# HanielUlises/GCN-GrabCut

Measured on AMD Instinct MI355X. Metric: images/sec end-to-end mask (DUTS-shape batch), higher is better.
Workload: dtype f32

## Files before the change

### gcn-grabcut_amd/csrc/ggc_internal.h

```cpp
#pragma once
#include <hip/hip_runtime.h>
#include <cstdint>
#include <cstdio>
#include <atomic>
#include <cstring>
#include <map>
#include <string>
#include <vector>
#include "../../include/ggc.h"
#include "../../include/ggc_fmath.h"

namespace ggc {

constexpr int WAVE = 64;

enum Slot : int {
    S_CSR_ROWPTR = 0, S_CSR_COL, S_CSR_EID, S_CSR_CURSOR, S_CSR_SCAN, S_DIS, S_BATCH, S_AGG_PACK,
    S_STATES, S_GATE, S_XW, S_AGG, S_SCORE, S_GVEC, S_HJK,
    S_PRE_A, S_PRE_B, S_PRE_C, S_PRE_D,
    S_SLIC_IMG, S_SLIC_TMP, S_SLIC_CENTERS, S_SLIC_DIST, S_SLIC_LABELS, S_SLIC_AUX,
    S_SLIC_AUX2, S_SLIC_AUX3, S_SLIC_AUX4, S_SLIC_MINMAX,
    S_G_STATS, S_G_FEAT, S_G_PAIRS, S_G_PAIRCNT, S_G_NL, S_G_EDGE_SRC, S_G_EDGE_DST,
    S_G_EDGE_ATTR, S_G_PTR, S_G_PRIOR, S_G_AUX, S_G_AUX2, S_G_AUX3, S_G_X,
    S_T_A, S_T_B, S_T_C,
    S_GC_A, S_GC_B, S_GC_C, S_GC_D, S_GC_E, S_GC_F, S_GC_G, S_GC_H, S_GC_I, S_GC_J,
    S_GC_K, S_GC_L, S_GC_M,
    S_CC_A, S_CC_B, S_CC_C,
    S_MISC_A, S_MISC_B,
    S_CLICK,
    S_MATTE, S_MATTE_MEAN, S_CFMATTE,
    S_FOREGROUND, S_FOREGROUND_VEC,
    S_MATTE_EVAL,
    S_FULLCUT,
    S_GEODESIC,
    S_STROKES,
    S_COUNT
};

struct Buf {
    void*  p = nullptr;
    size_t bytes = 0;
};

struct WeightSet {
    int D = 0;
    int Dt = 0;
    int n_layers = 0;
    int Q = 0, C = 0;
    int heads = 0;
    std::map<std::string, std::vector<float>> host;
    std::map<std::string, Buf> dev;
    bool dev_ok = false;
};

struct GraphState {
    int B = 0, H = 0, W = 0;
    int64_t n_total = 0, e_total = 0;
    std::vector<int64_t> node_ptr, edge_ptr;
    int64_t max_pairs = 0;
    int n_max = 0;
    const int32_t* n_nodes_dev = nullptr;
    bool valid = false;
};

}

namespace ggc {
struct ProfRec { const char* name; hipEvent_t a, b; };
}

struct ggc_ctx {
    int device = 0;
    std::string err;
    int prof_on = 0;
    double prof_overhead_ms = 0.0;
    std::vector<ggc::ProfRec> prof;
    std::vector<hipEvent_t> prof_pool;
    ggc::Buf slots[ggc::S_COUNT];
    ggc::WeightSet resgcn, gcnnet, gat;
    ggc::GraphState graph;
    int n_cu = 256;
    float prior_two_ce2 = (float)(2 * 0.45 * 0.45), prior_two_cs2 = (float)(2 * 0.40 * 0.40);
    int32_t* h_pinned = nullptr;
    static constexpr int H_PINNED_INTS = 4096;
};

namespace ggc {

struct Knobs {
    int mf_trace;
    int mf_warm;
    int mf_async_push_active;
    int mf_async_tile;
    int mf_async_hops;
    int mf_async_sweeps;
    int mf_dense_launches0, mf_dense_launches;
    int mf_dense_sweeps;
    int mf_relax_dense;
    int mf_partial_rounds;
    int agg_direct;
    int slic_seq_connectivity;
    int matte_eval_levels;
};
const Knobs& knobs();

int set_err(ggc_ctx* ctx, int code, const char* fmt, ...);
int read_i32(ggc_ctx* ctx, hipStream_t st, const int32_t* dev, int n, std::vector<int32_t>& host);
void* scratch(ggc_ctx* ctx, int slot, size_t bytes);
int build_csr(ggc_ctx* ctx, hipStream_t st, int N, int E, const int32_t* src, const int32_t* dst,
              int32_t* row_ptr, int32_t* col, int32_t* eid, int32_t* cursor, float* dis);

#define GGC_HIP(ctx, expr)                                                          \
    do {                                                                            \
        hipError_t _e = (expr);                                                     \
        if (_e != hipSuccess)                                                       \
            return ggc::set_err((ctx), GGC_E_DEVICE, "%s failed: %s (%s:%d)", #expr, \
                                hipGetErrorString(_e), __FILE__, __LINE__);          \
    } while (0)

#define GGC_LAUNCH_CHECK(ctx)                                                        \
    do {                                                                            \
        hipError_t _e = hipGetLastError();                                          \
        if (_e != hipSuccess)                                                       \
            return ggc::set_err((ctx), GGC_E_DEVICE, "kernel launch failed: %s (%s:%d)", \
                                hipGetErrorString(_e), __FILE__, __LINE__);          \
    } while (0)

#define GGC_REQUIRE(ctx, cond, code, ...)                      \
    do {                                                       \
        if (!(cond)) return ggc::set_err((ctx), (code), __VA_ARGS__); \
    } while (0)

template <typename T>
inline T* scratch_t(ggc_ctx* ctx, int slot, size_t count) {
    return reinterpret_cast<T*>(scratch(ctx, slot, count * sizeof(T)));
}

struct Carve {
    char* base = nullptr;
    size_t bytes = 0;
    template <typename T> T* take(size_t count) {
        T* p = base ? reinterpret_cast<T*>(base + bytes) : nullptr;
        bytes += (count * sizeof(T) + 255) & ~size_t(255);
        return p;
    }
};
template <typename Layout>
inline size_t carve_scratch(ggc_ctx* ctx, int slot, Layout&& layout) {
    Carve c;
    layout(c);
    c.base = static_cast<char*>(scratch(ctx, slot, c.bytes));
    if (!c.base) return 0;
    c.bytes = 0;
    layout(c);
    return c.bytes;
}

inline int cdiv(int64_t a, int64_t b) { return (int)((a + b - 1) / b); }

struct DeviceOnce {
    std::atomic<unsigned long long> mask{0};
    bool need(int dev) const { return dev < 0 || dev >= 64 || !((mask.load(std::memory_order_acquire) >> dev) & 1ull); }
    void done(int dev) { if (dev >= 0 && dev < 64) mask.fetch_or(1ull << dev, std::memory_order_release); }
};

struct ProfScope {
    ggc_ctx* ctx; hipStream_t st; hipEvent_t b = nullptr;
// ... 73 lines not shown
```

### gcn-grabcut_amd/csrc/ggc_math.h

```cpp
#pragma once
#include <hip/hip_runtime.h>
#include <cstdint>
#include <cstring>

namespace ggc {

__host__ __device__ inline double bits_to_double(uint64_t u) {
#if defined(__HIP_DEVICE_COMPILE__)
    return __longlong_as_double((long long)u);
#else
    double d; std::memcpy(&d, &u, 8); return d;
#endif
}
__host__ __device__ inline uint64_t double_to_bits(double d) {
#if defined(__HIP_DEVICE_COMPILE__)
    return (uint64_t)__double_as_longlong(d);
#else
    uint64_t u; std::memcpy(&u, &d, 8); return u;
#endif
}

__host__ __device__ inline double det_cbrt(double a) {
    double y = bits_to_double(double_to_bits(a) / 3 + 0x2A9F7893782DA1CEULL);
#pragma unroll
    for (int i = 0; i < 6; ++i) {
        const double y2 = y * y;
        y = y - (y2 * y - a) / (3.0 * y2);
    }
    return y;
}

__host__ __device__ inline double det_pow24(double a) {
    const double q = a * a;
    double y = bits_to_double(double_to_bits(q) / 5 + 0x3325FFFFFFFFFFFFULL);
#pragma unroll
    for (int i = 0; i < 7; ++i) {
        const double y2 = y * y;
        const double y4 = y2 * y2;
        y = y - (y4 * y - q) / (5.0 * y4);
    }
    return q * y;
}

__host__ __device__ inline double det_exp(double x) {
    const double LN2_HI = 6.93147180369123816490e-01, LN2_LO = 1.90821492927058770002e-10;
    const double INV_LN2 = 1.44269504088896338700e+00;
    if (x != x) return x;
    if (x < -745.2) return 0.0;
    if (x > 709.782712893384) return bits_to_double(0x7FF0000000000000ULL);
    const double k = rint(x * INV_LN2);
    const double r = (x - k * LN2_HI) - k * LN2_LO;
    double p = 1.0 / 6227020800.0;
    p = p * r + 1.0 / 479001600.0;
    p = p * r + 1.0 / 39916800.0;
    p = p * r + 1.0 / 3628800.0;
    p = p * r + 1.0 / 362880.0;
    p = p * r + 1.0 / 40320.0;
    p = p * r + 1.0 / 5040.0;
    p = p * r + 1.0 / 720.0;
    p = p * r + 1.0 / 120.0;
    p = p * r + 1.0 / 24.0;
    p = p * r + 1.0 / 6.0;
    p = p * r + 0.5;
    p = p * r + 1.0;
    p = p * r + 1.0;
    const long long ki = (long long)k;
    const long long k1 = ki / 2, k2 = ki - k1;
    return p * bits_to_double((uint64_t)(k1 + 1023) << 52) * bits_to_double((uint64_t)(k2 + 1023) << 52);
}

__host__ __device__ inline double det_log(double x) {
    const double LN2_HI = 6.93147180369123816490e-01, LN2_LO = 1.90821492927058770002e-10;
    if (x != x || x < 0.0) return bits_to_double(0x7FF8000000000000ULL);
    if (x == 0.0) return bits_to_double(0xFFF0000000000000ULL);
    if (x > 1.7976931348623157e308) return x;
    long long e = -1023;
    if (x < 2.2250738585072014e-308) { x = x * 18014398509481984.0; e -= 54; }
    const uint64_t u = double_to_bits(x);
    e += (long long)((u >> 52) & 0x7FF);
    double m = bits_to_double((u & 0x000FFFFFFFFFFFFFULL) | 0x3FF0000000000000ULL);
    if (m > 1.4142135623730951) { m = m * 0.5; e += 1; }
    const double f = m - 1.0;
    const double s = f / (2.0 + f);
    const double z = s * s;
    double q = 1.0 / 23.0;
    q = q * z + 1.0 / 21.0;
    q = q * z + 1.0 / 19.0;
    q = q * z + 1.0 / 17.0;
    q = q * z + 1.0 / 15.0;
    q = q * z + 1.0 / 13.0;
    q = q * z + 1.0 / 11.0;
    q = q * z + 1.0 / 9.0;
    q = q * z + 1.0 / 7.0;
    q = q * z + 1.0 / 5.0;
    q = q * z + 1.0 / 3.0;
    q = q * z + 1.0;
    const double de = (double)e;
    return de * LN2_HI + (de * LN2_LO + 2.0 * s * q);
}

}
```

### gcn-grabcut_amd/csrc/ggc_preprocess.hip

```cpp
#include "ggc_internal.h"
#include "ggc_math.h"

namespace ggc {

__device__ __forceinline__ double lab_f(double t) {
    return t > 0.008856 ? det_cbrt(t) : 7.787 * t + 16.0 / 116.0;
}

__device__ __forceinline__ int reflect101(int i, int n) {
    if (n == 1) return 0;
    if (i < 0) i = -i;
    if (i >= n) i = 2 * n - 2 - i;
    return i;
}

__device__ __forceinline__ float gray_at(const uint8_t* __restrict__ img, int W, int y, int x) {
    const uint8_t* p = img + ((size_t)y * W + x) * 3;
    return (float)((p[0] * 3735 + p[1] * 19235 + p[2] * 9798 + (1 << 14)) >> 15);
}

__global__ void __launch_bounds__(256) k_preprocess(int H, int W, const uint8_t* __restrict__ bgr,
                                                    const double* __restrict__ lut,
                                                    float* __restrict__ lab, float* __restrict__ hsv,
                                                    float* __restrict__ gray, float* __restrict__ grad) {
// ... 23 lines not shown
        double s = 0.0, h = 0.0;
        if (delta != 0.0) {
            s = delta / v;
            if (r == v) h = (g - b) / delta;
            if (g == v) h = 2.0 + (b - r) / delta;
            if (b == v) h = 4.0 + (r - g) / delta;
            h = h / 6.0;
            if (h < 0.0) h = h + 1.0;
        }
        hsv[3 * p + 0] = (float)h;
        hsv[3 * p + 1] = (float)s;
        hsv[3 * p + 2] = (float)v;
    }
    if (gray) gray[p] = (float)((b8 * 3735 + g8 * 19235 + r8 * 9798 + (1 << 14)) >> 15);
    if (grad) {
        const int ym = reflect101(y - 1, H), yp = reflect101(y + 1, H);
        const int xm = reflect101(x - 1, W), xp = reflect101(x + 1, W);
        const float a = gray_at(img, W, ym, xm), b = gray_at(img, W, ym, x), c = gray_at(img, W, ym, xp);
        const float d = gray_at(img, W, y, xm), f = gray_at(img, W, y, xp);
        const float g = gray_at(img, W, yp, xm), h = gray_at(img, W, yp, x), i = gray_at(img, W, yp, xp);
        const float gx = (c + 2.0f * f + i) - (a + 2.0f * d + g);
        const float gy = (g + 2.0f * h + i) - (a + 2.0f * b + c);
        grad[p] = sqrtf(gx * gx + gy * gy);
    }
}

}

namespace ggc {
__global__ void __launch_bounds__(256) k_convert_color8(size_t n, const uint8_t* __restrict__ bgr, int mode,
                                                        const double* __restrict__ lut, const int32_t* __restrict__ sdiv,
                                                        const int32_t* __restrict__ hdiv, uint8_t* __restrict__ out) {
    const size_t p = (size_t)blockIdx.x * blockDim.x + threadIdx.x;
    if (p >= n) return;
    const int b = bgr[3 * p + 0], g = bgr[3 * p + 1], r = bgr[3 * p + 2];
    if (mode == 0) {
        const int v = max(max(b, g), r), vmin = min(min(b, g), r), diff = v - vmin;
        const int s = (diff * sdiv[v] + (1 << 11)) >> 12;
        int h = (v == r) ? (g - b) : (v == g) ? (b - r + 2 * diff) : (r - g + 4 * diff);
        h = (h * hdiv[diff] + (1 << 11)) >> 12;
        if (h < 0) h += 180;
        out[3 * p + 0] = (uint8_t)h; out[3 * p + 1] = (uint8_t)s; out[3 * p + 2] = (uint8_t)v;
        return;
    }
    const double R = lut[r], G = lut[g], B = lut[b];
    const double X = R * 0.412453 + G * 0.357580 + B * 0.180423;
    const double Y = R * 0.212671 + G * 0.715160 + B * 0.072169;
    const double Z = R * 0.019334 + G * 0.119193 + B * 0.950227;
    const double tx = X / 0.95047, ty = Y / 1.0, tz = Z / 1.08883;
    const double fx = tx > 0.008856 ? det_cbrt(tx) : 7.787 * tx + 16.0 / 116.0;
    const double fy = ty > 0.008856 ? det_cbrt(ty) : 7.787 * ty + 16.0 / 116.0;
    const double fz = tz > 0.008856 ? det_cbrt(tz) : 7.787 * tz + 16.0 / 116.0;
    const double v[3] = {(116.0 * fy - 16.0) * 255.0 / 100.0, 500.0 * (fx - fy) + 128.0, 200.0 * (fy - fz) + 128.0};
#pragma unroll
    for (int c = 0; c < 3; ++c) {
        double q = floor(v[c] + 0.5);
        q = q < 0.0 ? 0.0 : (q > 255.0 ? 255.0 : q);
        out[3 * p + c] = (uint8_t)q;
    }
}
}

using namespace ggc;

extern "C" int ggc_preprocess(ggc_ctx* ctx, ggc_stream stream, int B, int H, int W, const uint8_t* bgr,
                              float* lab, float* hsv, float* gray, float* grad) {
    if (!ctx) return GGC_E_INVALID_ARG;
    GGC_REQUIRE(ctx, B >= 1 && H >= 1 && W >= 1, GGC_E_SHAPE, "bad shape B=%d H=%d W=%d", B, H, W);
    GGC_REQUIRE(ctx, bgr != nullptr, GGC_E_INVALID_ARG, "bgr is NULL");
    GGC_REQUIRE(ctx, B <= 65535, GGC_E_SHAPE, "batch %d exceeds the grid z limit", B);
    GGC_HIP(ctx, hipSetDevice(ctx->device));
    hipStream_t st = reinterpret_cast<hipStream_t>(stream);
    double* lut = scratch_t<double>(ctx, S_PRE_A, 256);
    if (!lut) return GGC_E_OOM;
    static thread_local double host_lut[256];
    static thread_local bool lut_ready = false;
    if (!lut_ready) {
        for (int u = 0; u < 256; ++u) {
            const double v = (double)u * (1.0 / 255.0);
            host_lut[u] = v > 0.04045 ? det_pow24((v + 0.055) / 1.055) : v / 12.92;
        }
        lut_ready = true;
    }
    GGC_HIP(ctx, hipMemcpyAsync(lut, host_lut, sizeof(host_lut), hipMemcpyHostToDevice, st));
    hipLaunchKernelGGL(k_preprocess, dim3(cdiv(W, 64), cdiv(H, 4), B), dim3(256), 0, st, H, W, bgr, lut, lab, hsv,
                       gray, grad);
    GGC_LAUNCH_CHECK(ctx);
    return GGC_OK;
}

extern "C" int ggc_convert_color8(ggc_ctx* ctx, ggc_stream stream, int64_t n_pixels, const uint8_t* bgr, int mode, uint8_t* out) {
    if (!ctx) return GGC_E_INVALID_ARG;
    GGC_REQUIRE(ctx, n_pixels >= 1 && bgr && out, GGC_E_INVALID_ARG, "bad arguments");
    GGC_REQUIRE(ctx, mode == 0 || mode == 1, GGC_E_INVALID_ARG, "mode %d: 0 = HSV, 1 = Lab", mode);
    GGC_HIP(ctx, hipSetDevice(ctx->device));
    hipStream_t st = reinterpret_cast<hipStream_t>(stream);
    double* lut = scratch_t<double>(ctx, S_PRE_A, 256);
    int32_t* tabs = scratch_t<int32_t>(ctx, S_PRE_B, 512);
    if (!lut || !tabs) return GGC_E_OOM;
    double host_lut[256];
    int32_t host_tabs[512];
    for (int u = 0; u < 256; ++u) {
        const double v = (double)u * (1.0 / 255.0);
        host_lut[u] = v > 0.04045 ? det_pow24((v + 0.055) / 1.055) : v / 12.92;
        host_tabs[u] = u ? (int32_t)rint((double)(255 << 12) / (double)u) : 0;
        host_tabs[256 + u] = u ? (int32_t)rint((double)(180 << 12) / (6.0 * (double)u)) : 0;
    }
    GGC_HIP(ctx, hipMemcpyAsync(lut, host_lut, sizeof(host_lut), hipMemcpyHostToDevice, st));
    GGC_HIP(ctx, hipMemcpyAsync(tabs, host_tabs, sizeof(host_tabs), hipMemcpyHostToDevice, st));
    GGC_HIP(ctx, hipStreamSynchronize(st));
    hipLaunchKernelGGL(k_convert_color8, dim3(cdiv((size_t)n_pixels, 256)), dim3(256), 0, st, (size_t)n_pixels, bgr, mode, lut, tabs,
                       tabs + 256, out);
    GGC_LAUNCH_CHECK(ctx);
    return GGC_OK;
}
```

### gcn-grabcut_amd/csrc/ggc_slic.hip

```cpp
#include "ggc_internal.h"
#include "ggc_math.h"
#include <cmath>
#include <vector>

namespace ggc {

__device__ __forceinline__ uint32_t f2ord(float f) {
    const uint32_t u = __float_as_uint(f);
    return (u & 0x80000000u) ? ~u : (u | 0x80000000u);
}
__device__ __forceinline__ float ord2f(uint32_t o) {
    return __uint_as_float((o & 0x80000000u) ? (o & 0x7FFFFFFFu) : ~o);
}

__global__ void k_minmax_init(int B, uint32_t* mm) {
    const int i = blockIdx.x * blockDim.x + threadIdx.x;
    if (i < B) { mm[2 * i] = 0xFFFFFFFFu; mm[2 * i + 1] = 0u; }
}

__global__ void __launch_bounds__(256) k_minmax(size_t n, const float* __restrict__ img, uint32_t* mm) {
    const float* im = img + (size_t)blockIdx.y * n;
    float lo = INFINITY, hi = -INFINITY;
    for (size_t i = (size_t)blockIdx.x * blockDim.x + threadIdx.x; i < n; i += (size_t)gridDim.x * blockDim.x) {
        const float v = im[i];
        lo = fminf(lo, v); hi = fmaxf(hi, v);
    }
    for (int o = 32; o > 0; o >>= 1) { lo = fminf(lo, __shfl_xor(lo, o, 64)); hi = fmaxf(hi, __shfl_xor(hi, o, 64)); }
    __shared__ float s_lo[4], s_hi[4];
    if ((threadIdx.x & 63) == 0) { s_lo[threadIdx.x >> 6] = lo; s_hi[threadIdx.x >> 6] = hi; }
    __syncthreads();
    if (threadIdx.x == 0) {
        lo = fminf(fminf(s_lo[0], s_lo[1]), fminf(s_lo[2], s_lo[3]));
        hi = fmaxf(fmaxf(s_hi[0], s_hi[1]), fmaxf(s_hi[2], s_hi[3]));
        atomicMin(&mm[2 * blockIdx.y], f2ord(lo));
        atomicMax(&mm[2 * blockIdx.y + 1], f2ord(hi));
    }
}

__global__ void __launch_bounds__(256) k_lab2(size_t P, const float* __restrict__ img,
                                              const uint32_t* __restrict__ mm, int rescale,
                                              float* __restrict__ out) {
    const size_t p = (size_t)blockIdx.x * blockDim.x + threadIdx.x;
    if (p >= P) return;
    const size_t base = ((size_t)blockIdx.y * P + p) * 3;
    const float mn = ord2f(mm[2 * blockIdx.y]), mx = ord2f(mm[2 * blockIdx.y + 1]);
    const float range = mx - mn;
    float lin[3];
#pragma unroll
    for (int c = 0; c < 3; ++c) {
        float v = img[base + c];
        if (rescale) { v = v - mn; if (mx != mn) v = v / range; }
        lin[c] = v > (float)0.04045 ? (float)det_pow24((double)((v + (float)0.055) / (float)1.055))
                                    : v / (float)12.92;
    }
    const float X = (lin[0] * (float)0.412453 + lin[1] * (float)0.357580) + lin[2] * (float)0.180423;
    const float Y = (lin[0] * (float)0.212671 + lin[1] * (float)0.715160) + lin[2] * (float)0.072169;
    const float Z = (lin[0] * (float)0.019334 + lin[1] * (float)0.119193) + lin[2] * (float)0.950227;
    const float t[3] = {X / (float)0.95047, Y / 1.0f, Z / (float)1.08883};
    float f[3];
#pragma unroll
    for (int c = 0; c < 3; ++c)
        f[c] = t[c] > (float)0.008856 ? (float)det_cbrt((double)t[c]) : (float)7.787 * t[c] + (float)(16.0 / 116.0);
    out[base + 0] = 116.0f * f[1] - 16.0f;
    out[base + 1] = 500.0f * (f[0] - f[1]);
    out[base + 2] = 200.0f * (f[1] - f[2]);
}

constexpr int MAX_RADIUS = 16;
struct GaussW { double w[2 * MAX_RADIUS + 1]; int r; };

__device__ __forceinline__ int reflect_sym(int i, int n) {
    if ((unsigned)i < (unsigned)n) return i;
    if (n == 1) return 0;
    const int period = 2 * n;
    i %= period; if (i < 0) i += period;
    return i < n ? i : period - 1 - i;
}

template <int AXIS, int R>
__global__ void __launch_bounds__(256) k_gauss(int H, int W, const float* __restrict__ in, GaussW g,
                                               float scale, int apply_scale, float* __restrict__ out) {
    const int col = blockIdx.x * 256 + threadIdx.x;
    if (col >= 3 * W) return;
    const int y = blockIdx.y;
    const size_t n = (size_t)H * W * 3;
    const float* im = in + (size_t)blockIdx.z * n;
    const int x = col / 3, c = col - 3 * x;
    const int l = AXIS == 0 ? y : x;
    const int len = AXIS == 0 ? H : W;
    auto at = [&](int idx) -> double {
        const int j = reflect_sym(idx, len);
        return (double)(AXIS == 0 ? im[((size_t)j * W + x) * 3 + c] : im[((size_t)y * W + j) * 3 + c]);
    };
    double tmp;
    if (R > 0) {
        constexpr int RR = R > 0 ? R : 1;
        double lo[RR], hi[RR];
        const double mid = at(l);
#pragma unroll
        for (int k = 0; k < R; ++k) { lo[k] = at(l - R + k); hi[k] = at(l + R - k); }
        tmp = mid * g.w[R];
#pragma unroll
        for (int k = 0; k < R; ++k) tmp += (lo[k] + hi[k]) * g.w[k];
    } else {
        tmp = at(l) * g.w[g.r];
        for (int jj = -g.r; jj < 0; ++jj) tmp += (at(l + jj) + at(l - jj)) * g.w[jj + g.r];
    }
    float v = (float)tmp;
    if (apply_scale) v = v * scale;
    out[(size_t)blockIdx.z * n + (size_t)y * W * 3 + col] = v;
}

constexpr int GV_ROWS = 20;
template <int R>
__global__ void __launch_bounds__(256) k_gauss_v(int H, int W, const float* __restrict__ in, GaussW g, float* __restrict__ out) {
    const int col = blockIdx.x * 256 + threadIdx.x;
    if (col >= 3 * W) return;
    const size_t n = (size_t)H * W * 3;
    const float* im = in + (size_t)blockIdx.z * n + col;
    float* o = out + (size_t)blockIdx.z * n + col;
    const int y0 = blockIdx.y * GV_ROWS;
    double v[2 * R + 1];
#pragma unroll
    for (int j = 0; j < 2 * R; ++j) v[j + 1] = (double)im[(size_t)reflect_sym(y0 - R + j, H) * W * 3];
#pragma unroll 4
    for (int y = y0; y < min(y0 + GV_ROWS, H); ++y) {
#pragma unroll
        for (int j = 0; j < 2 * R; ++j) v[j] = v[j + 1];
        v[2 * R] = (double)im[(size_t)reflect_sym(y + R, H) * W * 3];
        double tmp = v[R] * g.w[R];
#pragma unroll
        for (int k = 0; k < R; ++k) tmp += (v[k] + v[2 * R - k]) * g.w[k];
        o[(size_t)y * W * 3] = (float)tmp;
    }
}

__global__ void __launch_bounds__(256) k_scale(size_t n, const float* __restrict__ in, float scale,
                                               float* __restrict__ out) {
    const size_t i = (size_t)blockIdx.x * blockDim.x + threadIdx.x;
    if (i < n) out[i] = in[i] * scale;
}

struct SlicGeom {
    int H, W, K;
    int ny, nx, start_y, start_x, step_y, step_x;
    int win_y, win_x;
    float sw;
};

__device__ __forceinline__ int4 slic_window(float cy, float cx, const SlicGeom& g) {
    if (cy != cy || cx != cx) return make_int4(0, 0, 0, 0);
    float fy0 = cy - (float)(2 * g.win_y); if (!(fy0 > 0.0f)) fy0 = 0.0f;
    float fy1 = cy + (float)(2 * g.win_y) + 1.0f; if (!(fy1 < (float)g.H)) fy1 = (float)g.H;
    float fx0 = cx - (float)(2 * g.win_x); if (!(fx0 > 0.0f)) fx0 = 0.0f;
    float fx1 = cx + (float)(2 * g.win_x) + 1.0f; if (!(fx1 < (float)g.W)) fx1 = (float)g.W;
    return make_int4((int)fy0, (int)fy1, (int)fx0, (int)fx1);
}

__global__ void k_init_centers(SlicGeom g, float* __restrict__ centers, int4* __restrict__ bounds) {
    const int k = blockIdx.x * blockDim.x + threadIdx.x;
    if (k >= g.K) return;
    const size_t o = (size_t)blockIdx.y * g.K + k;
    const float cy = (float)(g.start_y + (k / g.nx) * g.step_y);
    const float cx = (float)(g.start_x + (k % g.nx) * g.step_x);
    centers[o * 5 + 0] = cy; centers[o * 5 + 1] = cx;
    centers[o * 5 + 2] = 0.0f; centers[o * 5 + 3] = 0.0f; centers[o * 5 + 4] = 0.0f;
    bounds[o] = slic_window(cy, cx, g);
}

struct Cand { int k, y0, y1, x0, x1; float cy, cx, c0, c1, c2; };

constexpr int TILE_W = 32, TILE_H = 16;

typedef float v2f __attribute__((ext_vector_type(2)));

__global__ void __launch_bounds__(256) k_slic_assign(SlicGeom g, const float* __restrict__ image,
                                                     const float* __restrict__ centers,
                                                     const int4* __restrict__ bounds,
                                                     int32_t* __restrict__ labels, int32_t* __restrict__ stale) {
    __shared__ Cand cand[256];
    __shared__ int wcount[4];
    const int tid = threadIdx.x, lane = tid & 63, wave = tid >> 6;
    const int b = blockIdx.z;
    const int tx0 = blockIdx.x * TILE_W, ty0 = blockIdx.y * TILE_H;
    const int px = tx0 + (wave & 1) * 16 + (lane & 15), pya = ty0 + (wave >> 1) * 8 + (lane >> 4), pyb = pya + 4;
    const bool ina = px < g.W && pya < g.H, inb = px < g.W && pyb < g.H;
    const size_t P = (size_t)g.H * g.W;
    const size_t pa = (size_t)b * P + (size_t)pya * g.W + px, pb = pa + (size_t)4 * g.W;
    v2f i0 = 0.f, i1 = 0.f, i2 = 0.f;
    if (ina) { i0.x = image[3 * pa]; i1.x = image[3 * pa + 1]; i2.x = image[3 * pa + 2]; }
    if (inb) { i0.y = image[3 * pb]; i1.y = image[3 * pb + 1]; i2.y = image[3 * pb + 2]; }
    const v2f fy = {(float)pya, (float)pyb};
    const float fx = (float)px;
    float best_a = INFINITY, best_b = INFINITY;
    int lab_a = -1, lab_b = -1;
    const float* cen = centers + (size_t)b * g.K * 5;
    const int4* bnd = bounds + (size_t)b * g.K;
    for (int base = 0; base < g.K; base += 256) {
        const int k = base + tid;
        bool hit = false;
        int4 bd = make_int4(0, 0, 0, 0);
        if (k < g.K) {
            bd = bnd[k];
            hit = bd.x < ty0 + TILE_H && bd.y > ty0 && bd.z < tx0 + TILE_W && bd.w > tx0 && bd.y > bd.x && bd.w > bd.z;
        }
        const unsigned long long bal = __ballot(hit);
        const int pre = __popcll(bal & ((1ull << lane) - 1ull));
        if (lane == 0) wcount[wave] = __popcll(bal);
        __syncthreads();
        int off = 0, total = 0;
#pragma unroll
        for (int w = 0; w < 4; ++w) { if (w < wave) off += wcount[w]; total += wcount[w]; }
        if (hit) {
            Cand c;
            c.k = k; c.y0 = bd.x; c.y1 = bd.y; c.x0 = bd.z; c.x1 = bd.w;
            c.cy = cen[k * 5 + 0]; c.cx = cen[k * 5 + 1];
// ... 399 lines not shown
    return g;
}

}

using namespace ggc;

static int enforce_connectivity(ggc_ctx* ctx, hipStream_t st, int B, int H, int W, const int32_t* raw, int min_size,
                                int max_size, int32_t* segments, int32_t* n_nodes) {
    const size_t P = (size_t)H * W;
    if (knobs().slic_seq_connectivity) {
        int32_t* queue = scratch_t<int32_t>(ctx, S_SLIC_AUX3, (size_t)B * (size_t)std::max(max_size, 1));
        if (!queue) return GGC_E_OOM;
        GGC_HIP(ctx, hipMemsetAsync(segments, 0xFF, sizeof(int32_t) * (size_t)B * P, st));
        ProfScope prof(ctx, st, "slic_connectivity");
        hipLaunchKernelGGL(k_connectivity_seq, dim3(B), dim3(64), 0, st, H, W, raw, min_size, max_size, queue, segments,
                           n_nodes);
        GGC_LAUNCH_CHECK(ctx);
        return GGC_OK;
    }
    {
        ProfScope prof(ctx, st, "slic_connectivity");
        const size_t BP = (size_t)B * P;
        const CnDims cd{B, H, W, (int)P, min_size, std::max(max_size, 1)};
        int32_t* work = scratch_t<int32_t>(ctx, S_SLIC_AUX3, BP * 6 + (size_t)B * (size_t)cd.max_size + 2 * (size_t)B + 16);
        uint8_t* pending = scratch_t<uint8_t>(ctx, S_SLIC_AUX4, BP);
        if (!work || !pending) return GGC_E_OOM;
        int32_t *parent = work, *csize = work + BP, *rank = work + 2 * BP, *tgt = work + 3 * BP, *mark = work + 4 * BP;
        int32_t* queue = work + 5 * BP;
        int32_t* qtop = work + 6 * BP + (size_t)B * cd.max_size;
        int32_t* n_big = qtop + B;
        GGC_HIP(ctx, hipMemsetAsync(pending, 1, BP, st));
        GGC_HIP(ctx, hipMemsetAsync(mark, 0, sizeof(int32_t) * BP, st));
        const dim3 g1(cdiv(BP, 256)), g2(cdiv(W, 64), cdiv(H, 4), B), g64(cdiv(BP, 64));
        for (int round = 0; round < 4096; ++round) {
            GGC_HIP(ctx, hipMemsetAsync(qtop, 0, sizeof(int32_t) * (B + 1), st));
            hipLaunchKernelGGL(k_cn_reset, g1, dim3(256), 0, st, cd, raw, pending, parent, csize);
            hipLaunchKernelGGL(k_cn_merge, g2, dim3(256), 0, st, cd, raw, pending, parent);
            hipLaunchKernelGGL(k_cn_size, g1, dim3(256), 0, st, cd, raw, pending, parent, csize);
            hipLaunchKernelGGL(k_cn_settle, g1, dim3(256), 0, st, cd, pending, parent, csize, n_big);
            GGC_LAUNCH_CHECK(ctx);
            int32_t h_big = 0;
            GGC_HIP(ctx, hipMemcpyAsync(&h_big, n_big, sizeof(int32_t), hipMemcpyDeviceToHost, st));
            GGC_HIP(ctx, hipStreamSynchronize(st));
            if (h_big == 0) break;
            hipLaunchKernelGGL(k_cn_carve, g64, dim3(64), 0, st, cd, round + 1, pending, parent, csize, mark, queue, qtop);
            GGC_LAUNCH_CHECK(ctx);
        }
        hipLaunchKernelGGL(k_cn_kept, g1, dim3(256), 0, st, cd, parent, csize, rank);
        hipLaunchKernelGGL(k_cn_scan, dim3(B), dim3(1024), 0, st, cd, rank, n_nodes);
        GGC_HIP(ctx, hipMemsetAsync(qtop, 0, sizeof(int32_t) * (B + 1), st));
        hipLaunchKernelGGL(k_cn_small, g64, dim3(64), 0, st, cd, 0x7FFFFFFF, parent, csize, mark, queue, qtop, tgt);
        hipLaunchKernelGGL(k_cn_write, g1, dim3(256), 0, st, cd, parent, csize, rank, tgt, segments);
        GGC_LAUNCH_CHECK(ctx);
    }
    return GGC_OK;
}

extern "C" int ggc_slic(ggc_ctx* ctx, ggc_stream stream, int B, int H, int W, const float* image,
                        int n_segments, float compactness, float sigma, int rescale_input,
                        int32_t* segments, int32_t* n_nodes) {
    if (!ctx) return GGC_E_INVALID_ARG;
    GGC_REQUIRE(ctx, B >= 1 && H >= 1 && W >= 1 && B <= 65535, GGC_E_SHAPE, "bad shape B=%d H=%d W=%d", B, H, W);
    GGC_REQUIRE(ctx, image && segments && n_nodes, GGC_E_INVALID_ARG, "null pointer");
    GGC_REQUIRE(ctx, n_segments >= 1 && compactness > 0.0f && sigma >= 0.0f, GGC_E_INVALID_ARG,
                "bad SLIC parameters n_segments=%d compactness=%g sigma=%g", n_segments, compactness, sigma);
    GGC_REQUIRE(ctx, (size_t)H * W < (1u << 30), GGC_E_SHAPE, "image too large");
    GGC_HIP(ctx, hipSetDevice(ctx->device));
    hipStream_t st = reinterpret_cast<hipStream_t>(stream);
    const size_t P = (size_t)H * W;

    const Grid seed = regular_grid(H, W, n_segments);
    GGC_REQUIRE(ctx, seed.K >= 1, GGC_E_SHAPE, "no SLIC seeds for %dx%d with n_segments=%d", H, W, n_segments);
    const Grid win = regular_grid(H, W, seed.K);
    SlicGeom g{};
    g.H = H; g.W = W; g.K = seed.K;
    g.ny = seed.ny; g.nx = seed.nx; g.start_y = seed.start_y; g.start_x = seed.start_x;
    g.step_y = seed.step_y; g.step_x = seed.step_x;
    g.win_y = win.step_y; g.win_x = win.step_x;
    const float step = (float)std::max(std::max(seed.step_y, seed.step_x), 1);
    g.sw = (float)(1.0 / (double)(step * step));

    float* img_a = scratch_t<float>(ctx, S_SLIC_IMG, (size_t)B * P * 3);
    float* img_b = scratch_t<float>(ctx, S_SLIC_TMP, (size_t)B * P * 3);
    uint32_t* mm = scratch_t<uint32_t>(ctx, S_SLIC_MINMAX, (size_t)B * 2);
    float* centers = scratch_t<float>(ctx, S_SLIC_CENTERS, (size_t)B * g.K * 5);
    int4* bounds = scratch_t<int4>(ctx, S_SLIC_AUX, (size_t)B * g.K);
    int32_t* raw = scratch_t<int32_t>(ctx, S_SLIC_LABELS, (size_t)B * P);
    int32_t* stale = scratch_t<int32_t>(ctx, S_SLIC_AUX2, (size_t)B * 10);
    if (!img_a || !img_b || !mm || !centers || !bounds || !raw || !stale) return GGC_E_OOM;

    hipLaunchKernelGGL(k_minmax_init, dim3(cdiv(B, 256)), dim3(256), 0, st, B, mm);
    hipLaunchKernelGGL(k_minmax, dim3(std::min(cdiv(P * 3, 256 * 8), 48), B), dim3(256), 0, st, P * 3, image, mm);
    hipLaunchKernelGGL(k_lab2, dim3(cdiv(P, 256), B), dim3(256), 0, st, P, image, mm, rescale_input, img_a);
    GGC_LAUNCH_CHECK(ctx);
    const float ratio = (float)(1.0 / (double)compactness);
    const float* km_img = nullptr;
    if (sigma > 0.0f) {
        GaussW gw{};
        gw.r = (int)(4.0 * (double)sigma + 0.5);
        GGC_REQUIRE(ctx, gw.r <= MAX_RADIUS, GGC_E_UNSUPPORTED, "sigma=%g needs radius %d > %d", sigma, gw.r, MAX_RADIUS);
        ggc_gaussian_taps((double)sigma, gw.r, gw.w);
        const double sum = np_pairwise_sum(gw.w, 2 * gw.r + 1);
        for (int i = 0; i < 2 * gw.r + 1; ++i) gw.w[i] = gw.w[i] / sum;
        GGC_REQUIRE(ctx, H <= 65535, GGC_E_SHAPE, "H=%d exceeds the launch grid", H);
        const dim3 grid(cdiv((size_t)W * 3, 256), H, B);
        if (gw.r == 4) {
            hipLaunchKernelGGL((k_gauss_v<4>), dim3(cdiv((size_t)W * 3, 256), cdiv(H, GV_ROWS), B), dim3(256), 0, st, H, W, img_a, gw, img_b);
            hipLaunchKernelGGL((k_gauss<1, 4>), grid, dim3(256), 0, st, H, W, img_b, gw, ratio, 1, img_a);
        } else {
            hipLaunchKernelGGL((k_gauss<0, 0>), grid, dim3(256), 0, st, H, W, img_a, gw, 1.0f, 0, img_b);
            hipLaunchKernelGGL((k_gauss<1, 0>), grid, dim3(256), 0, st, H, W, img_b, gw, ratio, 1, img_a);
        }
        km_img = img_a;
    } else {
        hipLaunchKernelGGL(k_scale, dim3(cdiv((size_t)B * P * 3, 256)), dim3(256), 0, st, (size_t)B * P * 3, img_a,
                           ratio, img_b);
        km_img = img_b;
    }
    GGC_LAUNCH_CHECK(ctx);
    hipLaunchKernelGGL(k_init_centers, dim3(cdiv(g.K, 256), B), dim3(256), 0, st, g, centers, bounds);
    GGC_HIP(ctx, hipMemsetAsync(raw, 0, sizeof(int32_t) * (size_t)B * P, st));
    GGC_HIP(ctx, hipMemsetAsync(stale, 0, sizeof(int32_t) * (size_t)B * 10, st));
    for (int it = 0; it < 10; ++it) {
        {
            ProfScope prof(ctx, st, "slic_assign");
            hipLaunchKernelGGL(k_slic_assign, dim3(cdiv(W, TILE_W), cdiv(H, TILE_H), B), dim3(256), 0, st, g, km_img,
                               centers, bounds, raw, stale + (size_t)it * B);
        }
        if (it < 9) {
            ProfScope prof(ctx, st, "slic_update");
            hipLaunchKernelGGL(k_slic_update, dim3(cdiv(g.K, 4 * UPD_GROUPS), B), dim3(256), 0, st, g, km_img, raw,
                               stale + (size_t)it * B, centers, bounds);
        }
        GGC_LAUNCH_CHECK(ctx);
    }
    const double seg_size = (double)P / (double)g.K;
    const int min_size = (int)(0.5 * seg_size), max_size = (int)(3.0 * seg_size);
    return enforce_connectivity(ctx, st, B, H, W, raw, min_size, max_size, segments, n_nodes);
}

namespace ggc {

__global__ void __launch_bounds__(256) k_minmax_u8(size_t n, const uint8_t* __restrict__ img, int32_t* __restrict__ mm) {
    const uint8_t* im = img + (size_t)blockIdx.y * n;
    int lo = 255, hi = 0;
    for (size_t i = (size_t)blockIdx.x * blockDim.x + threadIdx.x; i < n; i += (size_t)gridDim.x * blockDim.x) {
        const int v = im[i];
        lo = min(lo, v); hi = max(hi, v);
    }
    for (int o = 32; o > 0; o >>= 1) { lo = min(lo, __shfl_xor(lo, o, 64)); hi = max(hi, __shfl_xor(hi, o, 64)); }
    if ((threadIdx.x & 63) == 0) { atomicMin(&mm[2 * blockIdx.y], lo); atomicMax(&mm[2 * blockIdx.y + 1], hi); }
}
__global__ void k_minmax_u8_init(int B, int32_t* mm) {
    const int i = blockIdx.x * blockDim.x + threadIdx.x;
    if (i < B) { mm[2 * i] = 255; mm[2 * i + 1] = 0; }
}

__global__ void __launch_bounds__(256) k_rgb_lab64(size_t P, const uint8_t* __restrict__ bgr, const int32_t* __restrict__ mm,
                                                   GaussW g, int smooth, double* __restrict__ out) {
    const size_t p = (size_t)blockIdx.x * blockDim.x + threadIdx.x;
    if (p >= P) return;
    const size_t base = ((size_t)blockIdx.y * P + p) * 3;
    const double mn = (double)mm[2 * blockIdx.y], mx = (double)mm[2 * blockIdx.y + 1];
    const double range = mx - mn;
    double lin[3];
#pragma unroll
    for (int c = 0; c < 3; ++c) {
        double v = (double)bgr[base + 2 - c];
        v = v - mn; if (mx != mn) v = v / range;
        lin[c] = v > 0.04045 ? det_pow24((v + 0.055) / 1.055) : v / 12.92;
    }
    const double X = (lin[0] * 0.412453 + lin[1] * 0.357580) + lin[2] * 0.180423;
    const double Y = (lin[0] * 0.212671 + lin[1] * 0.715160) + lin[2] * 0.072169;
    const double Z = (lin[0] * 0.019334 + lin[1] * 0.119193) + lin[2] * 0.950227;
    const double t[3] = {X / 0.95047, Y / 1.0, Z / 1.08883};
    double f[3];
#pragma unroll
    for (int c = 0; c < 3; ++c) f[c] = t[c] > 0.008856 ? det_cbrt(t[c]) : 7.787 * t[c] + 16.0 / 116.0;
    double lab[3] = {116.0 * f[1] - 16.0, 500.0 * (f[0] - f[1]), 200.0 * (f[1] - f[2])};
    if (smooth) {
#pragma unroll
        for (int c = 0; c < 3; ++c) {
            double tmp = lab[c] * g.w[g.r];
            for (int jj = -g.r; jj < 0; ++jj) tmp += (lab[c] + lab[c]) * g.w[jj + g.r];
            lab[c] = tmp;
        }
    }
    out[base + 0] = lab[0]; out[base + 1] = lab[1]; out[base + 2] = lab[2];
}

template <int AXIS>
__global__ void __launch_bounds__(256) k_gauss64(int H, int W, const double* __restrict__ in, GaussW g, double scale,
                                                 int apply_scale, double* __restrict__ out) {
    const int col = blockIdx.x * 256 + threadIdx.x;
    if (col >= 3 * W) return;
    const int y = blockIdx.y;
    const size_t n = (size_t)H * W * 3;
    const double* im = in + (size_t)blockIdx.z * n;
    const int x = col / 3, c = col - 3 * x;
    const int l = AXIS == 0 ? y : x;
// ... 227 lines not shown
```

Before: 3739.

## Fuse Lab conversion with separable Gaussian, cache preprocess LUT upload, faster cbrt/pow

Replaces the separate Lab conversion, vertical blur and horizontal blur kernels with one kernel for the radius-4 case. It converts pixels to Lab on the fly, keeps a rolling vertical window in registers and does the horizontal pass through shared memory, which removes two full-image intermediate round trips and two launches. It also uploads the preprocess LUT only once per context instead of on every call, and adds in-range float versions of cbrt and pow(2.4) that run fewer Newton iterations. The trade-offs are halo recomputation in the fused kernel, one extra stream sync on the first call, and possible small numeric differences from the new math paths.

```diff
diff --git a/gcn-grabcut_amd/csrc/ggc_internal.h b/gcn-grabcut_amd/csrc/ggc_internal.h
--- a/gcn-grabcut_amd/csrc/ggc_internal.h
+++ b/gcn-grabcut_amd/csrc/ggc_internal.h
@@ -83,6 +83,7 @@
     float prior_two_ce2 = (float)(2 * 0.45 * 0.45), prior_two_cs2 = (float)(2 * 0.40 * 0.40);
     int32_t* h_pinned = nullptr;
     static constexpr int H_PINNED_INTS = 4096;
+    std::atomic<bool> pre_lut_ready{false};
 };
 
 namespace ggc {
diff --git a/gcn-grabcut_amd/csrc/ggc_math.h b/gcn-grabcut_amd/csrc/ggc_math.h
--- a/gcn-grabcut_amd/csrc/ggc_math.h
+++ b/gcn-grabcut_amd/csrc/ggc_math.h
@@ -40,6 +40,39 @@
         y = y - (y4 * y - q) / (5.0 * y4);
     }
     return q * y;
+}
+
+constexpr float DET_CBRT_F32_LO = 0.008856f, DET_CBRT_F32_HI = 1.25f;
+constexpr float DET_POW24_F32_LO = 0.05f, DET_POW24_F32_HI = 1.0f;
+
+__host__ __device__ inline float det_cbrt_f32(float t) {
+    if (!(t >= DET_CBRT_F32_LO && t <= DET_CBRT_F32_HI)) return (float)det_cbrt((double)t);
+    const double a = (double)t;
+    double r = bits_to_double(0x553F09FC49D9B000ULL - double_to_bits(a) / 3);
+#pragma unroll
+    for (int i = 0; i < 3; ++i) {
+        const double e = 1.0 - a * (r * r * r);
+        r = r + (r * e) * (1.0 / 3.0);
+    }
+    const double r2 = r * r;
+    const double y = a * r2;
+    return (float)(y - ((y * y * y - a) * r2) * (1.0 / 3.0));
+}
+
+__host__ __device__ inline float det_pow24_f32(float t) {
+    if (!(t >= DET_POW24_F32_LO && t <= DET_POW24_F32_HI)) return (float)det_pow24((double)t);
+    const double q = (double)t * (double)t;
+    double s = bits_to_double(0x4CB8BC2FDC10B800ULL - double_to_bits(q) / 5);
+#pragma unroll
+    for (int i = 0; i < 3; ++i) {
+        const double s2 = s * s;
+        const double e = 1.0 - q * ((s2 * s2) * s);
+        s = s + (s * e) * (1.0 / 5.0);
+    }
+    const double s2 = s * s, s4 = s2 * s2;
+    const double y = q * s4;
+    const double y2 = y * y;
+    return (float)(q * (y - (((y2 * y2) * y - q) * s4) * (1.0 / 5.0)));
 }
 
 __host__ __device__ inline double det_exp(double x) {
diff --git a/gcn-grabcut_amd/csrc/ggc_preprocess.hip b/gcn-grabcut_amd/csrc/ggc_preprocess.hip
--- a/gcn-grabcut_amd/csrc/ggc_preprocess.hip
+++ b/gcn-grabcut_amd/csrc/ggc_preprocess.hip
@@ -129,7 +129,11 @@
         }
         lut_ready = true;
     }
-    GGC_HIP(ctx, hipMemcpyAsync(lut, host_lut, sizeof(host_lut), hipMemcpyHostToDevice, st));
+    if (!ctx->pre_lut_ready.load(std::memory_order_acquire)) {
+        GGC_HIP(ctx, hipMemcpyAsync(lut, host_lut, sizeof(host_lut), hipMemcpyHostToDevice, st));
+        GGC_HIP(ctx, hipStreamSynchronize(st));
+        ctx->pre_lut_ready.store(true, std::memory_order_release);
+    }
     hipLaunchKernelGGL(k_preprocess, dim3(cdiv(W, 64), cdiv(H, 4), B), dim3(256), 0, st, H, W, bgr, lut, lab, hsv,
                        gray, grad);
     GGC_LAUNCH_CHECK(ctx);
diff --git a/gcn-grabcut_amd/csrc/ggc_slic.hip b/gcn-grabcut_amd/csrc/ggc_slic.hip
--- a/gcn-grabcut_amd/csrc/ggc_slic.hip
+++ b/gcn-grabcut_amd/csrc/ggc_slic.hip
@@ -37,6 +37,28 @@
     }
 }
 
+__device__ __forceinline__ void lab2_pixel(const float (&px)[3], float mn, float mx, int rescale, float (&lab)[3]) {
+    const float range = mx - mn;
+    float lin[3];
+#pragma unroll
+    for (int c = 0; c < 3; ++c) {
+        float v = px[c];
+        if (rescale) { v = v - mn; if (mx != mn) v = v / range; }
+        lin[c] = v > (float)0.04045 ? det_pow24_f32((v + (float)0.055) / (float)1.055) : v / (float)12.92;
+    }
+    const float X = (lin[0] * (float)0.412453 + lin[1] * (float)0.357580) + lin[2] * (float)0.180423;
+    const float Y = (lin[0] * (float)0.212671 + lin[1] * (float)0.715160) + lin[2] * (float)0.072169;
+    const float Z = (lin[0] * (float)0.019334 + lin[1] * (float)0.119193) + lin[2] * (float)0.950227;
+    const float t[3] = {X / (float)0.95047, Y / 1.0f, Z / (float)1.08883};
+    float f[3];
+#pragma unroll
+    for (int c = 0; c < 3; ++c)
+        f[c] = t[c] > (float)0.008856 ? det_cbrt_f32(t[c]) : (float)7.787 * t[c] + (float)(16.0 / 116.0);
+    lab[0] = 116.0f * f[1] - 16.0f;
+    lab[1] = 500.0f * (f[0] - f[1]);
+    lab[2] = 200.0f * (f[1] - f[2]);
+}
+
 __global__ void __launch_bounds__(256) k_lab2(size_t P, const float* __restrict__ img,
                                               const uint32_t* __restrict__ mm, int rescale,
                                               float* __restrict__ out) {
@@ -44,26 +66,10 @@
     if (p >= P) return;
     const size_t base = ((size_t)blockIdx.y * P + p) * 3;
     const float mn = ord2f(mm[2 * blockIdx.y]), mx = ord2f(mm[2 * blockIdx.y + 1]);
-    const float range = mx - mn;
-    float lin[3];
-#pragma unroll
-    for (int c = 0; c < 3; ++c) {
-        float v = img[base + c];
-        if (rescale) { v = v - mn; if (mx != mn) v = v / range; }
-        lin[c] = v > (float)0.04045 ? (float)det_pow24((double)((v + (float)0.055) / (float)1.055))
-                                    : v / (float)12.92;
-    }
-    const float X = (lin[0] * (float)0.412453 + lin[1] * (float)0.357580) + lin[2] * (float)0.180423;
-    const float Y = (lin[0] * (float)0.212671 + lin[1] * (float)0.715160) + lin[2] * (float)0.072169;
-    const float Z = (lin[0] * (float)0.019334 + lin[1] * (float)0.119193) + lin[2] * (float)0.950227;
-    const float t[3] = {X / (float)0.95047, Y / 1.0f, Z / (float)1.08883};
-    float f[3];
-#pragma unroll
-    for (int c = 0; c < 3; ++c)
-        f[c] = t[c] > (float)0.008856 ? (float)det_cbrt((double)t[c]) : (float)7.787 * t[c] + (float)(16.0 / 116.0);
-    out[base + 0] = 116.0f * f[1] - 16.0f;
-    out[base + 1] = 500.0f * (f[0] - f[1]);
-    out[base + 2] = 200.0f * (f[1] - f[2]);
+    const float px[3] = {img[base], img[base + 1], img[base + 2]};
+    float lab[3];
+    lab2_pixel(px, mn, mx, rescale, lab);
+    out[base + 0] = lab[0]; out[base + 1] = lab[1]; out[base + 2] = lab[2];
 }
 
 constexpr int MAX_RADIUS = 16;
@@ -77,7 +83,7 @@
     return i < n ? i : period - 1 - i;
 }
 
-template <int AXIS, int R>
+template <int AXIS>
 __global__ void __launch_bounds__(256) k_gauss(int H, int W, const float* __restrict__ in, GaussW g,
                                                float scale, int apply_scale, float* __restrict__ out) {
     const int col = blockIdx.x * 256 + threadIdx.x;
@@ -92,46 +98,67 @@
         const int j = reflect_sym(idx, len);
         return (double)(AXIS == 0 ? im[((size_t)j * W + x) * 3 + c] : im[((size_t)y * W + j) * 3 + c]);
     };
-    double tmp;
-    if (R > 0) {
-        constexpr int RR = R > 0 ? R : 1;
-        double lo[RR], hi[RR];
-        const double mid = at(l);
-#pragma unroll
-        for (int k = 0; k < R; ++k) { lo[k] = at(l - R + k); hi[k] = at(l + R - k); }
-        tmp = mid * g.w[R];
-#pragma unroll
-        for (int k = 0; k < R; ++k) tmp += (lo[k] + hi[k]) * g.w[k];
-    } else {
-        tmp = at(l) * g.w[g.r];
-        for (int jj = -g.r; jj < 0; ++jj) tmp += (at(l + jj) + at(l - jj)) * g.w[jj + g.r];
-    }
+    double tmp = at(l) * g.w[g.r];
+    for (int jj = -g.r; jj < 0; ++jj) tmp += (at(l + jj) + at(l - jj)) * g.w[jj + g.r];
     float v = (float)tmp;
     if (apply_scale) v = v * scale;
     out[(size_t)blockIdx.z * n + (size_t)y * W * 3 + col] = v;
 }
 
-constexpr int GV_ROWS = 20;
-template <int R>
-__global__ void __launch_bounds__(256) k_gauss_v(int H, int W, const float* __restrict__ in, GaussW g, float* __restrict__ out) {
-    const int col = blockIdx.x * 256 + threadIdx.x;
-    if (col >= 3 * W) return;
+constexpr int FG_R = 4, FG_THREADS = 128, FG_TX = FG_THREADS - 2 * FG_R, FG_ROWS = 60;
+__global__ void __launch_bounds__(FG_THREADS) k_lab2_gauss4(int H, int W, const float* __restrict__ img,
+                                                            const uint32_t* __restrict__ mm, int rescale, GaussW g,
+                                                            float scale, float* __restrict__ out) {
+    __shared__ float s_row[2][FG_THREADS * 3];
+    const int tid = threadIdx.x;
+    const int tx0 = blockIdx.x * FG_TX, y0 = blockIdx.y * FG_ROWS, y1 = min(y0 + FG_ROWS, H);
     const size_t n = (size_t)H * W * 3;
-    const float* im = in + (size_t)blockIdx.z * n + col;
-    float* o = out + (size_t)blockIdx.z * n + col;
-    const int y0 = blockIdx.y * GV_ROWS;
-    double v[2 * R + 1];
-#pragma unroll
-    for (int j = 0; j < 2 * R; ++j) v[j + 1] = (double)im[(size_t)reflect_sym(y0 - R + j, H) * W * 3];
-#pragma unroll 4
-    for (int y = y0; y < min(y0 + GV_ROWS, H); ++y) {
-#pragma unroll
-        for (int j = 0; j < 2 * R; ++j) v[j] = v[j + 1];
-        v[2 * R] = (double)im[(size_t)reflect_sym(y + R, H) * W * 3];
-        double tmp = v[R] * g.w[R];
-#pragma unroll
-        for (int k = 0; k < R; ++k) tmp += (v[k] + v[2 * R - k]) * g.w[k];
-        o[(size_t)y * W * 3] = (float)tmp;
+    const float* im = img + (size_t)blockIdx.z * n;
+    float* o = out + (size_t)blockIdx.z * n;
+    const float mn = ord2f(mm[2 * blockIdx.z]), mx = ord2f(mm[2 * blockIdx.z + 1]);
+    const int xc = tx0 - FG_R + tid;
+    const bool need = xc < W + FG_R;
+    const float* col = im + (size_t)reflect_sym(xc, W) * 3;
+    double w[FG_R + 1];
+#pragma unroll
+    for (int k = 0; k <= FG_R; ++k) w[k] = g.w[k];
+    double v[2 * FG_R + 1][3];
+    float nxt[3] = {0.f, 0.f, 0.f};
+    if (need) { const float* p = col + (size_t)reflect_sym(y0 - FG_R, H) * W * 3; nxt[0] = p[0]; nxt[1] = p[1]; nxt[2] = p[2]; }
+    for (int r = y0 - FG_R; r < y1 + FG_R; ++r) {
+        const float px[3] = {nxt[0], nxt[1], nxt[2]};
+        if (need && r + 1 < y1 + FG_R) { const float* p = col + (size_t)reflect_sym(r + 1, H) * W * 3; nxt[0] = p[0]; nxt[1] = p[1]; nxt[2] = p[2]; }
+#pragma unroll
+        for (int j = 0; j < 2 * FG_R; ++j) { v[j][0] = v[j + 1][0]; v[j][1] = v[j + 1][1]; v[j][2] = v[j + 1][2]; }
+        if (need) {
+            float lab[3];
+            lab2_pixel(px, mn, mx, rescale, lab);
+            v[2 * FG_R][0] = (double)lab[0]; v[2 * FG_R][1] = (double)lab[1]; v[2 * FG_R][2] = (double)lab[2];
+        }
+        const int y = r - FG_R;
+        if (y < y0) continue;
+        float* s = s_row[y & 1];
+        if (need) {
+#pragma unroll
+            for (int c = 0; c < 3; ++c) {
+                double tmp = v[FG_R][c] * w[FG_R];
+#pragma unroll
+                for (int k = 0; k < FG_R; ++k) tmp += (v[k][c] + v[2 * FG_R - k][c]) * w[k];
+                s[tid * 3 + c] = (float)tmp;
+            }
+        }
+        __syncthreads();
+        float* orow = o + ((size_t)y * W + tx0) * 3;
+#pragma unroll
+        for (int i = 0; i < (FG_TX * 3 + FG_THREADS - 1) / FG_THREADS; ++i) {
+            const int e = tid + i * FG_THREADS;
+            if (e < FG_TX * 3 && tx0 * 3 + e < W * 3) {
+                double tmp = (double)s[e + 3 * FG_R] * w[FG_R];
+#pragma unroll
+                for (int k = 0; k < FG_R; ++k) tmp += ((double)s[e + 3 * k] + (double)s[e + 3 * (2 * FG_R - k)]) * w[k];
+                orow[e] = (float)tmp * scale;
+            }
+        }
     }
 }
 
@@ -697,41 +724,44 @@
     g.sw = (float)(1.0 / (double)(step * step));
 
     float* img_a = scratch_t<float>(ctx, S_SLIC_IMG, (size_t)B * P * 3);
-    float* img_b = scratch_t<float>(ctx, S_SLIC_TMP, (size_t)B * P * 3);
     uint32_t* mm = scratch_t<uint32_t>(ctx, S_SLIC_MINMAX, (size_t)B * 2);
     float* centers = scratch_t<float>(ctx, S_SLIC_CENTERS, (size_t)B * g.K * 5);
     int4* bounds = scratch_t<int4>(ctx, S_SLIC_AUX, (size_t)B * g.K);
     int32_t* raw = scratch_t<int32_t>(ctx, S_SLIC_LABELS, (size_t)B * P);
     int32_t* stale = scratch_t<int32_t>(ctx, S_SLIC_AUX2, (size_t)B * 10);
-    if (!img_a || !img_b || !mm || !centers || !bounds || !raw || !stale) return GGC_E_OOM;
-
-    hipLaunchKernelGGL(k_minmax_init, dim3(cdiv(B, 256)), dim3(256), 0, st, B, mm);
-    hipLaunchKernelGGL(k_minmax, dim3(std::min(cdiv(P * 3, 256 * 8), 48), B), dim3(256), 0, st, P * 3, image, mm);
-    hipLaunchKernelGGL(k_lab2, dim3(cdiv(P, 256), B), dim3(256), 0, st, P, image, mm, rescale_input, img_a);
-    GGC_LAUNCH_CHECK(ctx);
-    const float ratio = (float)(1.0 / (double)compactness);
-    const float* km_img = nullptr;
+    if (!img_a || !mm || !centers || !bounds || !raw || !stale) return GGC_E_OOM;
+
+    GaussW gw{};
     if (sigma > 0.0f) {
-        GaussW gw{};
         gw.r = (int)(4.0 * (double)sigma + 0.5);
         GGC_REQUIRE(ctx, gw.r <= MAX_RADIUS, GGC_E_UNSUPPORTED, "sigma=%g needs radius %d > %d", sigma, gw.r, MAX_RADIUS);
         ggc_gaussian_taps((double)sigma, gw.r, gw.w);
         const double sum = np_pairwise_sum(gw.w, 2 * gw.r + 1);
         for (int i = 0; i < 2 * gw.r + 1; ++i) gw.w[i] = gw.w[i] / sum;
         GGC_REQUIRE(ctx, H <= 65535, GGC_E_SHAPE, "H=%d exceeds the launch grid", H);
-        const dim3 grid(cdiv((size_t)W * 3, 256), H, B);
-        if (gw.r == 4) {
-            hipLaunchKernelGGL((k_gauss_v<4>), dim3(cdiv((size_t)W * 3, 256), cdiv(H, GV_ROWS), B), dim3(256), 0, st, H, W, img_a, gw, img_b);
-            hipLaunchKernelGGL((k_gauss<1, 4>), grid, dim3(256), 0, st, H, W, img_b, gw, ratio, 1, img_a);
+    }
+    const bool fused = sigma > 0.0f && gw.r == FG_R;
+    float* img_b = fused ? nullptr : scratch_t<float>(ctx, S_SLIC_TMP, (size_t)B * P * 3);
+    if (!fused && !img_b) return GGC_E_OOM;
+
+    const float ratio = (float)(1.0 / (double)compactness);
+    const float* km_img = img_a;
+    hipLaunchKernelGGL(k_minmax_init, dim3(cdiv(B, 256)), dim3(256), 0, st, B, mm);
+    hipLaunchKernelGGL(k_minmax, dim3(std::min(cdiv(P * 3, 256 * 8), 48), B), dim3(256), 0, st, P * 3, image, mm);
+    if (fused) {
+        hipLaunchKernelGGL(k_lab2_gauss4, dim3(cdiv(W, FG_TX), cdiv(H, FG_ROWS), B), dim3(FG_THREADS), 0, st, H, W, image, mm,
+                           rescale_input, gw, ratio, img_a);
+    } else {
+        hipLaunchKernelGGL(k_lab2, dim3(cdiv(P, 256), B), dim3(256), 0, st, P, image, mm, rescale_input, img_a);
+        if (sigma > 0.0f) {
+            const dim3 grid(cdiv((size_t)W * 3, 256), H, B);
+            hipLaunchKernelGGL((k_gauss<0>), grid, dim3(256), 0, st, H, W, img_a, gw, 1.0f, 0, img_b);
+            hipLaunchKernelGGL((k_gauss<1>), grid, dim3(256), 0, st, H, W, img_b, gw, ratio, 1, img_a);
         } else {
-            hipLaunchKernelGGL((k_gauss<0, 0>), grid, dim3(256), 0, st, H, W, img_a, gw, 1.0f, 0, img_b);
-            hipLaunchKernelGGL((k_gauss<1, 0>), grid, dim3(256), 0, st, H, W, img_b, gw, ratio, 1, img_a);
-        }
-        km_img = img_a;
-    } else {
-        hipLaunchKernelGGL(k_scale, dim3(cdiv((size_t)B * P * 3, 256)), dim3(256), 0, st, (size_t)B * P * 3, img_a,
-                           ratio, img_b);
-        km_img = img_b;
+            hipLaunchKernelGGL(k_scale, dim3(cdiv((size_t)B * P * 3, 256)), dim3(256), 0, st, (size_t)B * P * 3, img_a,
+                               ratio, img_b);
+            km_img = img_b;
+        }
     }
     GGC_LAUNCH_CHECK(ctx);
     hipLaunchKernelGGL(k_init_centers, dim3(cdiv(g.K, 256), B), dim3(256), 0, st, g, centers, bounds);
```

Result: no change. 3775 (median of 6 runs) (+1.0%).
